# jianing-sun/Mask-YOLO

Measured on AMD Instinct MI355X. Metric: images/sec fwd+bwd, 224x224 Shapes batch 32, at 1 MI355X, higher is better.
Workload: dtype f32

## Files before the change

### include/myolo_hip_internal.h

```cpp
#ifndef MYOLO_HIP_INTERNAL_H
#define MYOLO_HIP_INTERNAL_H

#include "myolo_hip.h"

#ifdef __cplusplus
extern "C" {
#endif

int myolo_bn_frozen_coeffs_batched(const float* params, const float* stats, const int64_t* table, int nlayers, float* coeffs,
                                   void* stream);

int myolo_bn_act_bwd_frozen_post(const float* dy, const float* a_post, const float* gamma, const float* beta, const float* scale,
                                 float* dx, float* dgamma, float* dbeta, int64_t M, int C, int act,
                                 void* ws, size_t ws_bytes, void* stream);

int myolo_wprep_create(void* arena, size_t arena_bytes, void** handle);
int myolo_wprep_destroy(void* h);
int myolo_wprep_activate(void* h);
int myolo_wprep_count(void* h);
int myolo_wprep_invalidate(void* h);
int myolo_wprep_refresh(void* h, int first, int last, int max_idle, void* stream);
int myolo_wprep_stats(void* h, long long* hits, long long* misses, long long* bytes_used);
int myolo_wprep_overflows(void* h, long long* n);

// ... 49 lines not shown
                                   float* dx, float* dgamma, float* dbeta, int64_t M, int C, int act, const double* part, int nblk,
                                   void* ws, size_t ws_bytes, void* stream);

size_t myolo_wino63_plane_elems(int N, int C);
size_t myolo_wino63_u_elems(int Cin, int Cout);

int myolo_wino63_weight_transform(const float* w, float* U, int Cin, int Cout, void* stream);
int myolo_wino63_multiply(const float* V, const float* U, float* M, int N, int Cin, int Cout, void* stream);
int myolo_wino63_multiply_w(const float* V, const float* w, float* U_scratch, float* M, int N, int Cin, int Cout, void* stream);
int myolo_wino63_input_transform(const float* x, const float* scale, const float* shift, int act,
                                 float* keep, const int32_t* keep_sel, int keep_cap,
                                 float* V, int N, int C, void* stream);
int myolo_wino63_boundary(const float* M, const float* bias, const float* scale, const float* shift, int act,
                          float* y, float* keep, int keep_pre, const int32_t* keep_sel, int keep_cap,
                          float* Vn, int N, int C, void* stream);
int myolo_wino63_input_transform_roialign(const float* feature, const float* boxes, const int32_t* box_ind, float* V, int B, int FH, int FW,
                                          int C, int nb, void* stream);
size_t myolo_wino63_output_transform_bn_ws_bytes(int N, int C);
int myolo_wino63_output_transform_bn_stats(const float* M, const float* bias, float* y, int N, int C, const float* gamma, const float* beta,
                                           float* mean, float* var, float* scale, float* shift, float* moving_mean, float* moving_var,
                                           void* ws, size_t ws_bytes, void* stream);
size_t myolo_wino63_bwd_weight_ws_bytes(int N, int Cin, int Cout);
int myolo_wino63_bwd_weight_lazybn(const float* v_saved, const float* y_pre, const float* dy_compact, const int32_t* inv, const float* scale,
                                   const float* shift, const float* ka, const float* kb, int act, float* dw, int N, int Cin, int Cout,
                                   void* ws, size_t ws_bytes, void* stream);
int myolo_wino63_lazybn_transforms(const float* y_pre, const float* dy_compact, const int32_t* inv, const float* scale, const float* shift,
                                   const float* ka, const float* kb, int act, float* V, float* Q, int N, int C, void* stream);
size_t myolo_wino63_bwd_data_from_v_ws_bytes(int N, int Cin, int Cout);
int myolo_wino63_bwd_data_from_v(const float* V, const float* w, float* dx, int N, int Cin, int Cout, void* ws, size_t ws_bytes, void* stream);
size_t myolo_wino63_bwd_weight_from_q_ws_bytes(int N, int Cin, int Cout);
int myolo_wino63_bwd_weight_from_q(const float* v_saved, const float* Q, float* dw, int N, int Cin, int Cout, void* ws, size_t ws_bytes,
                                   void* stream);

int myolo_gemm_tn_bf16x6_planes(const float* A, const float* B, float* C, int nruns, const int64_t* rows, const int32_t* nq, int Ka, int N,
                                void* ws, size_t ws_bytes, void* stream);
int myolo_deconv2x2s2_bwd_weight_bf16x6(const float* x, const float* dy, float* dw, int N, int H, int W, int Cin, int Cout, void* ws, size_t ws_bytes,
                                        void* stream);

size_t myolo_wino63_bwd_data_ws_bytes(int N, int Cin, int Cout);
int myolo_wino63_bwd_data_lazybn(const float* y_pre, const float* dy_compact, const int32_t* inv, const float* scale, const float* shift,
                                 const float* ka, const float* kb, int act, const float* w, float* dx, int N, int Cin, int Cout, void* ws,
                                 size_t ws_bytes, void* stream);
int myolo_conv3x3s2_c3_affine_act_fwd(const float* x, const float* w, const float* scale, const float* shift, int act, float* y,
                                      int N, int H, int W, int Cout, void* stream);
size_t myolo_conv3x3s2_c3_bnstats_ws_bytes(int N, int H, int W, int Cout);
int myolo_conv3x3s2_c3_bnstats_fwd(const float* x, const float* w, float* y, const float* gamma, const float* beta, float* mean, float* var,
                                   float* scale, float* shift, float* moving_mean, float* moving_var, int N, int H, int W, int Cout, int phases,
                                   void* ws, size_t ws_bytes, void* stream);
size_t myolo_dwconv3x3_bnstats_ws_bytes(int N, int H, int W, int C, int stride);
int myolo_dwconv3x3_bnstats_fwd(const float* x, const float* in_scale, const float* in_shift, int in_act, const float* w, float* y,
                                const float* gamma, const float* beta, float* mean, float* var, float* scale, float* shift,
                                float* moving_mean, float* moving_var, int N, int H, int W, int C, int stride, int phases,
                                void* ws, size_t ws_bytes, void* stream);
int myolo_dwconv3x3_bwd_weight_affine_in(const float* x, const float* in_scale, const float* in_shift, int in_act, const float* dy, float* dw,
                                         int N, int H, int W, int C, int stride, void* ws, size_t ws_bytes, void* stream);
int    myolo_pwconv1x1_bnstats_ok(int Cin, int Cout);
size_t myolo_pwconv1x1_bnstats_ws_bytes(int64_t M, int Cin, int Cout);
int myolo_pwconv1x1_bnstats_fwd(const float* x, const float* in_scale, const float* in_shift, int in_act, const float* w, float* y,
                                const float* gamma, const float* beta, float* mean, float* var, float* scale, float* shift,
                                float* moving_mean, float* moving_var, int64_t M, int Cin, int Cout, int phases, void* ws, size_t ws_bytes, void* stream);
int myolo_pwconv1x1_bwd_weight_affine_in(const float* x, const float* in_scale, const float* in_shift, int in_act, const float* dy, float* dw,
                                         int64_t M, int Cin, int Cout, void* ws, size_t ws_bytes, void* stream);

int myolo_mask_bce_sel(const float* target_masks, const int32_t* target_class_ids, const float* pred, float loss_weight,
                       float* loss_out, float* dz_sel, int NR, int h, int w, int C, void* ws, size_t ws_bytes, void* stream);
size_t myolo_mask_head_out_bwd_sel_ws_bytes(int NR, int Cin);
// ... 128 lines not shown
```

### mask-yolo_amd/csrc/mem_kernels.hip

```cpp
#include "myolo_common.h"
#include <type_traits>
#include <stdlib.h>
#include <stdarg.h>
#include <string.h>

static thread_local char g_err[512] = "";
extern "C" void myolo_set_error(const char* fmt, ...)
{
    va_list ap;
    va_start(ap, fmt);
    vsnprintf(g_err, sizeof(g_err), fmt, ap);
    va_end(ap);
}
extern "C" const char* myolo_last_error_string(void) { return g_err; }
extern "C" int myolo_version(void) { return 213; }

static MyoloOptions default_options() { MyoloOptions o = {}; o.bn_fused_tf_variance = 1; o.tn_wgs = 224; return o; }
MyoloOptions g_myolo_opt = default_options();
static int* option_slot(const char* name)
{
    static const struct { const char* n; int MyoloOptions::*m; } tab[] = {
        {"gemm_generic", &MyoloOptions::gemm_generic}, {"no_splitk", &MyoloOptions::no_splitk}, {"bf16_no256", &MyoloOptions::bf16_no256},
        {"bf16_force256", &MyoloOptions::bf16_force256}, {"bf16_no_c3", &MyoloOptions::bf16_no_c3}, {"bf16_no_loopn", &MyoloOptions::bf16_no_loopn},
        {"bf16_mask_valu", &MyoloOptions::bf16_mask_valu}, {"bf16_mask_nofin", &MyoloOptions::bf16_mask_nofin},
        {"deconv_mask_legacy", &MyoloOptions::deconv_mask_legacy}, {"crop_bf16_legacy", &MyoloOptions::crop_bf16_legacy},
        {"tune0", &MyoloOptions::tune0}, {"wino_x6", &MyoloOptions::wino_x6}, {"wino_no_bt", &MyoloOptions::wino_no_bt},
        {"wino_no_mixed", &MyoloOptions::wino_no_mixed}, {"x6_no_half_tiles", &MyoloOptions::x6_no_half_tiles},
        {"w63_legacy", &MyoloOptions::w63_legacy}, {"pw_x6_min_rows", &MyoloOptions::pw_x6_min_rows}, {"deconv_no_x6", &MyoloOptions::deconv_no_x6},
        {"pw_no_smallm", &MyoloOptions::pw_no_smallm}, {"pw_no_x6", &MyoloOptions::pw_no_x6}, {"tn_no_x6", &MyoloOptions::tn_no_x6},
        {"tn_wgs", &MyoloOptions::tn_wgs}, {"tn_x6_legacy", &MyoloOptions::tn_x6_legacy}, {"no_trunk_fusion", &MyoloOptions::no_trunk_fusion},
        {"bn_fused_tf_variance", &MyoloOptions::bn_fused_tf_variance},
    };
    if (!name) return nullptr;
    for (const auto& e : tab)
        if (strcmp(e.n, name) == 0) return &(g_myolo_opt.*(e.m));
    return nullptr;
}
extern "C" int myolo_set_option(const char* name, int value)
{
    int* s = option_slot(name);
    MYOLO_REQUIRE(s, "set_option: unknown option '%s'", name ? name : "(null)");
    *s = value;
    return MYOLO_OK;
}
extern "C" int myolo_get_option(const char* name, int* value)
{
    int* s = option_slot(name);
    MYOLO_REQUIRE(s && value, "get_option: unknown option '%s'", name ? name : "(null)");
    *value = *s;
    return MYOLO_OK;
}

#include <vector>
struct WPrepEntry {
    const void* w; int kind; long long d0, d1, d2;
    size_t off, bytes;
    unsigned long long gen;
    unsigned long long last_use;
    std::function<void(void*, hipStream_t)> run;
};
struct WPrep {
    char* arena; size_t cap, used;
    unsigned long long gen;
// ... 3439 lines not shown
```

### mask-yolo_amd/csrc/myolo_common.h

```cpp
#pragma once
#include <hip/hip_runtime.h>
#include <stdint.h>
#include <stdio.h>
#include "../../include/myolo_hip_internal.h"

extern "C" void myolo_set_error(const char* fmt, ...);

struct MyoloOptions {
    int gemm_generic;
    int no_splitk;
    int bf16_no256;
    int bf16_no_loopn;
    int bf16_mask_valu;
    int bf16_mask_nofin;
    int deconv_mask_legacy;
    int bf16_no_c3;
    int bf16_force256;
    int crop_bf16_legacy;
    int tune0;
    int wino_x6;
    int wino_no_bt;
    int wino_no_mixed;
    int x6_no_half_tiles;
    int w63_legacy;
    int pw_x6_min_rows;
    int deconv_no_x6;
    int pw_no_smallm;
    int pw_no_x6;
    int tn_no_x6;
    int tn_wgs;
    int tn_x6_legacy;
    int no_trunk_fusion;
    int bn_fused_tf_variance;
};
extern MyoloOptions g_myolo_opt;

#define MYOLO_REQUIRE(cond, ...)                                   \
    do {                                                           \
        if (!(cond)) {                                             \
            myolo_set_error(__VA_ARGS__);                          \
            return MYOLO_EINVAL;                                   \
        }                                                          \
    } while (0)

#define MYOLO_NEED_WS(bytes)                                                         \
    do {                                                                             \
        if ((size_t)(bytes) > ws_bytes || (ws == nullptr && (bytes) > 0)) {          \
            myolo_set_error("%s: workspace too small (%zu needed, %zu given)",       \
                            __func__, (size_t)(bytes), ws_bytes);                    \
            return MYOLO_EWORKSPACE;                                                 \
        }                                                                            \
    } while (0)

#define MYOLO_CHECK_LAUNCH()                                                         \
    do {                                                                             \
        hipError_t e__ = hipGetLastError();                                          \
        if (e__ != hipSuccess) {                                                     \
            myolo_set_error("%s: launch failed: %s", __func__, hipGetErrorString(e__)); \
            return MYOLO_ELAUNCH;                                                    \
        }                                                                            \
    } while (0)

#include <functional>
enum { WP_TRANSPOSE = 1, WP_X6_SPLIT = 2, WP_WINO63_U = 3, WP_WINO43_U = 4 };
// ... 47 lines not shown
```

### mask-yolo_amd/csrc/wino_mm.hip

```cpp
#include "myolo_common.h"

typedef float f32x16 __attribute__((ext_vector_type(16)));
typedef unsigned int u32x4 __attribute__((ext_vector_type(4)));

#define MM_BM 128
#define MM_BN 256
#define MM_BK 16
#define MM_LD 20
#define MM_OOB 0x7fffff00u

struct MMRun {
    long long rows;
    long long a_off;
    long long b_off;
    long long c_off;
    long long tile0;
    int mtiles;
    int nq;
};
struct MMArgs {
    const float* A;
    const float* Bt;
    float* C;
    int K, N;
// ... 994 lines not shown
        else hipLaunchKernelGGL(wino_mm_x6_kernel<MM_EP_PLAIN>, dim3((unsigned)tiles), dim3(256), 0, s, a);
    } else {
        if (!b_is_nk) {
            hipLaunchKernelGGL(mm_transpose_kn_kernel, dim3((N + 31) / 32, (K + 31) / 32), dim3(256), 0, s, B, (float*)ws, K, N);
            a.Bt = (const float*)ws;
        } else a.Bt = B;
        hipLaunchKernelGGL(wino_mm_kernel<MM_EP_PLAIN>, dim3((unsigned)tiles), dim3(256), 0, s, a);
    }
    MYOLO_CHECK_LAUNCH();
    return MYOLO_OK;
}

#define TN_T 256
struct TNRun {
    long long rows;
    long long a_off, b_off;
    long long rows_per_split;
    long long unit0;
    int plane0;
    int nq;
    int splits;
};
struct TNArgs {
    const float* a_scale;
    const float* a_shift;
    int a_act;
    int gH, gW, gCo;
    const float* A;
    const float* B;
    float* part;
    float* C;
    int Ka, N;
    int nruns;
    int tiles_k, tiles_n;
    long long nunits;
    long long unit_base;
    int tune;
    TNRun run[4];
};

template <bool AG = false, bool UNI = true>
__global__ __launch_bounds__(512, 1) void wino_tn_x6_kernel(TNArgs p)
{
    __shared__ __attribute__((aligned(16))) unsigned char Ls[2][2][TN_T * X6_REC];

    const int tid = threadIdx.x, lane = tid & 63, wave = tid >> 6;
    const int wm = wave >> 2, wn = wave & 3, half = lane >> 5, l31 = lane & 31;
    const int ntile = p.tiles_k * p.tiles_n;
  const long long bid = p.unit_base + blockIdx.x;
  {
    const long long pair = bid / ntile;
    const int tile = (int)(bid - pair * ntile);
    const int kat = tile / p.tiles_n, nt = tile - kat * p.tiles_n;
    int ri = 0;
#pragma unroll
    for (int k = 1; k < 4; ++k)
        if (k < p.nruns && pair >= p.run[k].unit0) ri = k;
    const TNRun& R = p.run[ri];
    const long long local = pair - R.unit0;
    const int z = (int)(local / R.splits), sp = (int)(local - (long long)z * R.splits);
    const long long r0 = (long long)sp * R.rows_per_split;
    long long r1 = r0 + R.rows_per_split;
    if (r1 > R.rows) r1 = R.rows;
    const long long nrows = r1 > r0 ? r1 - r0 : 0;
    const int nk = (int)((nrows + MM_BK - 1) / MM_BK);

// ... 116 lines not shown
                for (int pc = 0; pc < 3; ++pc) fn[pc] = *reinterpret_cast<const bf16x8*>(la + afr + (t + 1) * 32 * X6_REC + pc * 32);
            }
#ifdef MM_X6_TUNE
            if (!(p.tune & 4))
#endif
#pragma unroll
            for (int u = 0; u < 2; ++u) {
                acc[t][u] = __builtin_amdgcn_mfma_f32_32x32x16_bf16(fa[0], fb[u][2], acc[t][u], 0, 0, 0);
                acc[t][u] = __builtin_amdgcn_mfma_f32_32x32x16_bf16(fa[2], fb[u][0], acc[t][u], 0, 0, 0);
                acc[t][u] = __builtin_amdgcn_mfma_f32_32x32x16_bf16(fa[1], fb[u][1], acc[t][u], 0, 0, 0);
                acc[t][u] = __builtin_amdgcn_mfma_f32_32x32x16_bf16(fa[0], fb[u][1], acc[t][u], 0, 0, 0);
                acc[t][u] = __builtin_amdgcn_mfma_f32_32x32x16_bf16(fa[1], fb[u][0], acc[t][u], 0, 0, 0);
                acc[t][u] = __builtin_amdgcn_mfma_f32_32x32x16_bf16(fa[0], fb[u][0], acc[t][u], 0, 0, 0);
            }
            if (t == 0 && more) split_store(cur ^ 1, 0);
            if (t == 1 && more) split_store(cur ^ 1, 1);
            if (t == 2 && c + 2 < nk) gload();
            if (t < 3) { fa[0] = fn[0]; fa[1] = fn[1]; fa[2] = fn[2]; }
        }
        __syncthreads();
    }
    float* Pp = p.part + pair * (long long)p.Ka * p.N + ((long long)kat * TN_T + wm * 128) * p.N + nt * TN_T + wn * 64 + l31;
#pragma unroll
    for (int t = 0; t < 4; ++t)
#pragma unroll
        for (int r = 0; r < 16; ++r) {
            const int row = t * 32 + (r & 3) + 8 * (r >> 2) + 4 * half;
#pragma unroll
            for (int u = 0; u < 2; ++u) Pp[(long long)row * p.N + u * 32] = acc[t][u][r];
        }
  }
}

__global__ __launch_bounds__(256) void tn_x6_reduce_kernel(TNArgs p)
{
    const int plane = blockIdx.y;
    int ri = 0;
#pragma unroll
    for (int k = 1; k < 4; ++k)
        if (k < p.nruns && plane >= p.run[k].plane0) ri = k;
    const TNRun& R = p.run[ri];
    const long long n4 = (long long)p.Ka * p.N / 4;
    const long long i = (long long)blockIdx.x * 256 + threadIdx.x;
    if (i >= n4) return;
    const float4* src = reinterpret_cast<const float4*>(p.part) + (R.unit0 + (long long)(plane - R.plane0) * R.splits) * n4 + i;
    float4 s = make_float4(0.f, 0.f, 0.f, 0.f);
    int k = 0;
    for (; k + 4 <= R.splits; k += 4) {
        const float4 a = src[(long long)k * n4], b = src[(long long)(k + 1) * n4], c = src[(long long)(k + 2) * n4], d = src[(long long)(k + 3) * n4];
        s.x += a.x; s.y += a.y; s.z += a.z; s.w += a.w;
        s.x += b.x; s.y += b.y; s.z += b.z; s.w += b.w;
        s.x += c.x; s.y += c.y; s.z += c.z; s.w += c.w;
        s.x += d.x; s.y += d.y; s.z += d.z; s.w += d.w;
    }
    for (; k < R.splits; ++k) {
        const float4 a = src[(long long)k * n4];
        s.x += a.x; s.y += a.y; s.z += a.z; s.w += a.w;
    }
    reinterpret_cast<float4*>(p.C)[(long long)plane * n4 + i] = s;
}

bool myolo_gemm_tn_x6_ok(int Ka, int N) { return g_myolo_opt.wino_x6 && !g_myolo_opt.tn_no_x6 && Ka >= TN_T && (Ka % TN_T) == 0 && N >= TN_T && (N % TN_T) == 0; }

static long long tn_x6_plan(int nruns, const long long* rows, const int* nq, int Ka, int N, TNArgs* a)
{
    const int ntile = (Ka / TN_T) * (N / TN_T);
    long long total_rows = 0;
    for (int r = 0; r < nruns; ++r) total_rows += rows[r] * nq[r];
    const long long target_units = 3 * (g_myolo_opt.tn_wgs > 0 ? g_myolo_opt.tn_wgs : 256);
    long long rps = ((total_rows * ntile + target_units - 1) / target_units + MM_BK - 1) / MM_BK * MM_BK;
    if (rps < 8 * MM_BK) rps = 8 * MM_BK;
    long long pairs = 0;
    for (int iter = 0; iter < 64; ++iter) {
        pairs = 0;
        for (int r = 0; r < nruns; ++r) pairs += (long long)nq[r] * ((rows[r] + rps - 1) / rps);
        if (pairs * ntile <= target_units || rps >= total_rows) break;
        rps += MM_BK;
    }
    if (a) {
        long long unit = 0;
        int plane = 0;
        a->nruns = 0;
        for (int r = 0; r < nruns; ++r) {
            if (rows[r] <= 0 || nq[r] <= 0) continue;
            TNRun& R = a->run[a->nruns++];
            R.rows = rows[r]; R.nq = nq[r]; R.plane0 = plane; R.unit0 = unit;
            R.splits = (int)((rows[r] + rps - 1) / rps);
            R.rows_per_split = ((rows[r] + R.splits - 1) / R.splits + MM_BK - 1) / MM_BK * MM_BK;
            unit += (long long)R.nq * R.splits;
            plane += nq[r];
        }
    }
    return pairs;
}

static long long tn_x6_grid(long long nunits) { return g_myolo_opt.tn_wgs > 0 && nunits > g_myolo_opt.tn_wgs ? g_myolo_opt.tn_wgs : nunits; }

template <bool AG>
static void tn_x6_launch(TNArgs& a, hipStream_t s)
{
    for (long long base = 0, g = tn_x6_grid(a.nunits); base < a.nunits; base += g) {
        a.unit_base = base;
        const unsigned n = (unsigned)(a.nunits - base < g ? a.nunits - base : g);
        if (g_myolo_opt.tn_x6_legacy) hipLaunchKernelGGL((wino_tn_x6_kernel<AG, false>), dim3(n), dim3(512), 0, s, a);
        else hipLaunchKernelGGL((wino_tn_x6_kernel<AG, true>), dim3(n), dim3(512), 0, s, a);
    }
}

size_t myolo_gemm_tn_x6_ws_bytes(int nruns, const long long* rows, const int* nq, int Ka, int N)
{
    return align256((size_t)tn_x6_plan(nruns, rows, nq, Ka, N, nullptr) * Ka * N * sizeof(float));
}

int myolo_gemm_tn_x6_runs(const float* A, const float* B, float* C, int nruns, const long long* rows, const long long* a_off, const long long* b_off,
                          const int* nq, int Ka, int N, void* part, size_t part_bytes, hipStream_t s,
                          const float* a_scale, const float* a_shift, int a_act)
{
    if (nruns < 0 || nruns > 4 || Ka < TN_T || (Ka % TN_T) || N < TN_T || (N % TN_T) || ((uintptr_t)A & 15) || ((uintptr_t)B & 15) || ((uintptr_t)C & 15)) {
        myolo_set_error("gemm_tn_x6_runs: needs Ka %% %d == 0, N %% %d == 0, <= 4 runs, 16-byte aligned operands", TN_T, TN_T);
        return MYOLO_EINVAL;
    }
    TNArgs a{};
    a.A = A; a.B = B; a.C = C; a.part = (float*)part; a.Ka = Ka; a.N = N; a.tiles_k = Ka / TN_T; a.tiles_n = N / TN_T;
    a.a_scale = a_scale; a.a_shift = a_shift; a.a_act = a_act;
    const long long pairs = tn_x6_plan(nruns, rows, nq, Ka, N, &a);
    if ((size_t)pairs * Ka * N * sizeof(float) > part_bytes || !part) {
        myolo_set_error("gemm_tn_x6_runs: workspace too small (%zu needed, %zu given)", (size_t)pairs * Ka * N * sizeof(float), part_bytes);
        return MYOLO_EWORKSPACE;
    }
    int k = 0, planes = 0;
    for (int r = 0; r < nruns; ++r) {
        if (rows[r] <= 0 || nq[r] <= 0) continue;
        if ((a_off[r] | b_off[r]) & 3) { myolo_set_error("gemm_tn_x6_runs: run offsets must be multiples of 4 elements"); return MYOLO_EINVAL; }
        a.run[k].a_off = a_off[r]; a.run[k].b_off = b_off[r];
        planes += nq[r];
        ++k;
    }
    if (pairs <= 0) return MYOLO_OK;
    a.nunits = pairs * a.tiles_k * a.tiles_n;
#ifdef MM_X6_TUNE
    a.tune = g_myolo_opt.tune0;
#endif
    tn_x6_launch<false>(a, s);
    const long long n4 = (long long)Ka * N / 4;
    hipLaunchKernelGGL(tn_x6_reduce_kernel, dim3((unsigned)((n4 + 255) / 256), planes), dim3(256), 0, s, a);
    return MYOLO_OK;
}

extern "C" int myolo_gemm_tn_bf16x6_planes(const float* A, const float* B, float* C, int nruns, const int64_t* rows, const int32_t* nq, int Ka, int N,
                                           void* ws, size_t ws_bytes, void* stream)
{
    MYOLO_REQUIRE(A && B && C && rows && nq && nruns >= 0 && nruns <= 4 && Ka > 0 && N > 0, "gemm_tn_bf16x6_planes: bad arguments");
    long long r[4], ao[4], bo[4], at = 0;
    int q[4];
    for (int k = 0; k < nruns; ++k) {
        MYOLO_REQUIRE(rows[k] >= 0 && nq[k] >= 0, "gemm_tn_bf16x6_planes: negative run");
        r[k] = rows[k]; q[k] = nq[k]; ao[k] = at * Ka; bo[k] = at * N;
        at += rows[k] * nq[k];
    }
    const int rc = myolo_gemm_tn_x6_runs(A, B, C, nruns, r, ao, bo, q, Ka, N, ws, ws_bytes, (hipStream_t)stream);
    if (rc) return rc;
    MYOLO_CHECK_LAUNCH();
    return MYOLO_OK;
}

bool myolo_pw_x6_ok(int K, int N) { return g_myolo_opt.wino_x6 && !g_myolo_opt.pw_no_x6 && K >= 256 && (K % MM_BK) == 0 && (N % MM_BN) == 0; }
size_t myolo_pw_x6_split_bytes(int K, int N) { return align256((size_t)K * N * 6); }
int myolo_pw_x6_fwd(const float* x, const float* in_scale, const float* in_shift, int in_act, const float* w, float* y, double* stat,
                    long long M, int K, int N, void* split, hipStream_t s)
{
    MMArgs a{};
    a.A = x; a.C = y; a.K = K; a.N = N; a.nruns = 1;
    a.a_scale = in_scale; a.a_shift = in_shift; a.a_act = in_act; a.stat = stat;
#ifdef MM_X6_TUNE
    a.tune = g_myolo_opt.tune0;
#endif
    MMRun& R = a.run[0];
    R.rows = M; R.a_off = 0; R.b_off = 0; R.c_off = 0; R.nq = 1; R.tile0 = 0;
    R.mtiles = (int)((M + MM_BM - 1) / MM_BM);
// ... 15 lines not shown
{
    const int K = Cin, N = 4 * Co;
    MMArgs a{};
    a.A = x; a.C = y; a.K = K; a.N = N; a.nruns = 1; a.bias = bias; a.H = H; a.W = W; a.Co = Co; a.a_act = act;
#ifdef MM_X6_TUNE
    a.tune = g_myolo_opt.tune0;
#endif
    MMRun& R = a.run[0];
    R.rows = M; R.nq = 1; R.mtiles = (int)((M + MM_BM - 1) / MM_BM);
    a.Bt = x6_split_weights(w, split, K, N, 0, s);
    hipLaunchKernelGGL((wino_mm_x6_kernel<MM_EP_DECONV, false, MM_A_PLAIN>), dim3((unsigned)((long long)R.mtiles * (N / MM_BN))), dim3(256), 0, s, a);
    return MYOLO_OK;
}
int myolo_deconv_x6_bwd_data(const float* dy, const float* w, float* dx, long long M, int H, int W, int Cin, int Co, void* split, hipStream_t s)
{
    const int K = 4 * Co, N = Cin;
    MMArgs a{};
    a.A = dy; a.C = dx; a.K = K; a.N = N; a.nruns = 1; a.H = H; a.W = W; a.Co = Co;
#ifdef MM_X6_TUNE
    a.tune = g_myolo_opt.tune0;
#endif
    MMRun& R = a.run[0];
    R.rows = M; R.nq = 1; R.mtiles = (int)((M + MM_BM - 1) / MM_BM);
    a.Bt = x6_split_weights(w, split, K, N, 1, s);
    hipLaunchKernelGGL((wino_mm_x6_kernel<MM_EP_PLAIN, false, MM_A_DECONV>), dim3((unsigned)((long long)R.mtiles * (N / MM_BN))), dim3(256), 0, s, a);
    return MYOLO_OK;
}


size_t myolo_deconv_x6_bwd_weight_ws_bytes(long long M, int Cin, int Co)
{
    const long long rows[1] = {M};
    const int nq[1] = {1};
    return myolo_gemm_tn_x6_ws_bytes(1, rows, nq, 4 * Co, Cin);
}
int myolo_deconv_x6_bwd_weight(const float* x, const float* dy, float* dw, long long M, int H, int W, int Cin, int Co, void* part, size_t part_bytes,
                               hipStream_t s)
{
    const int Ka = 4 * Co, N = Cin;
    TNArgs a{};
    a.A = dy; a.B = x; a.C = dw; a.part = (float*)part; a.Ka = Ka; a.N = N; a.tiles_k = Ka / TN_T; a.tiles_n = N / TN_T;
    a.gH = H; a.gW = W; a.gCo = Co;
    const long long rows[1] = {M};
    const int nq[1] = {1};
    const long long pairs = tn_x6_plan(1, rows, nq, Ka, N, &a);
    if ((size_t)pairs * Ka * N * sizeof(float) > part_bytes || !part) {
        myolo_set_error("deconv_x6_bwd_weight: workspace too small (%zu needed, %zu given)", (size_t)pairs * Ka * N * sizeof(float), part_bytes);
        return MYOLO_EWORKSPACE;
    }
    a.run[0].a_off = 0; a.run[0].b_off = 0;
    a.nunits = pairs * a.tiles_k * a.tiles_n;
    tn_x6_launch<true>(a, s);
    const long long n4 = (long long)Ka * N / 4;
    hipLaunchKernelGGL(tn_x6_reduce_kernel, dim3((unsigned)((n4 + 255) / 256), 1), dim3(256), 0, s, a);
    return MYOLO_OK;
}

extern "C" int myolo_deconv2x2s2_bwd_weight_bf16x6(const float* x, const float* dy, float* dw, int N, int H, int W, int Cin, int Cout, void* ws, size_t ws_bytes,
                                                   void* stream)
{
    MYOLO_REQUIRE(x && dy && dw && N > 0 && H > 0 && W > 0 && Cin > 0 && Cout > 0 && (Cin % TN_T) == 0 && ((4 * Cout) % TN_T) == 0 &&
                  (((uintptr_t)x | (uintptr_t)dy | (uintptr_t)dw) & 15) == 0, "deconv2x2s2_bwd_weight_bf16x6: needs Cin %% 256 == 0, 4 Cout %% 256 == 0, 16-byte aligned operands");
    const int rc = myolo_deconv_x6_bwd_weight(x, dy, dw, (long long)N * H * W, H, W, Cin, Cout, ws, ws_bytes, (hipStream_t)stream);
    if (rc) return rc;
    MYOLO_CHECK_LAUNCH();
    return MYOLO_OK;
}
```

### mask-yolo_amd/myolo/_ext.py

```python
import ctypes
import os

import torch

_LIB = None
_HERE = os.path.dirname(os.path.abspath(__file__))
LIB_PATH = os.environ.get("MYOLO_LIB") or os.path.join(_HERE, "_lib", "libmyolo_hip.so")

P, I, L, F, Z, D = ctypes.c_void_p, ctypes.c_int, ctypes.c_int64, ctypes.c_float, ctypes.c_size_t, ctypes.c_double

SIGS = {
    "myolo_conv3x3s2_c3_fwd": [P, P, P, I, I, I, I, P],
    "myolo_conv3x3s2_c3_affine_act_fwd": [P, P, P, P, I, P, I, I, I, I, P],
    "myolo_conv3x3s2_c3_bwd_weight": [P, P, P, I, I, I, I, P, Z, P],
    "myolo_dwconv3x3_fwd": [P, P, P, I, I, I, I, I, P],
    "myolo_dwconv3x3_affine_act_fwd": [P, P, P, P, I, P, I, I, I, I, I, P],
    "myolo_dwconv3x3_bwd_data": [P, P, P, I, I, I, I, I, P],
    "myolo_dwconv3x3_bwd_data_bnsums": [P, P, P, I, I, I, I, I, P, P, P, P, P, I, P, I, P],
    "myolo_bn_act_bwd_from_partials": [P, P, P, P, P, P, P, P, P, L, I, I, P, I, P, Z, P],
    "myolo_dwconv3x3_bwd_weight": [P, P, P, I, I, I, I, I, P, Z, P],
    "myolo_pwconv1x1_fwd": [P, P, P, P, L, I, I, P, Z, P],
    "myolo_pwconv1x1_affine_act_fwd": [P, P, P, P, I, P, L, I, I, P, Z, P],
    "myolo_bn_frozen_coeffs_batched": [P, P, P, I, P, P],
    "myolo_pwconv1x1_bwd_data": [P, P, P, L, I, I, P, Z, P],
# ... 120 lines not shown
}


def load():
    global _LIB
    if _LIB is not None:
        return _LIB
    if not os.path.exists(LIB_PATH):
        raise RuntimeError("libmyolo_hip.so not built (%s): run `python __graft_entry__.py` "
                           "(hipcc --offload-arch=gfx950); there is no fallback path" % LIB_PATH)
    lib = ctypes.CDLL(LIB_PATH)
    for name, argtypes in SIGS.items():
        fn = getattr(lib, name)
        fn.argtypes = argtypes
        fn.restype = ctypes.c_int
    lib.myolo_version.restype = ctypes.c_int
    lib.myolo_last_error_string.restype = ctypes.c_char_p
    lib.myolo_workspace_bytes.argtypes = [L, I, I]
    lib.myolo_workspace_bytes.restype = Z
    lib.myolo_conv3x3_wino_ws_bytes.argtypes = [I, I, I, I, I, I]
    lib.myolo_conv3x3_wino_ws_bytes.restype = Z
    lib.myolo_matmul_f32_ws_bytes.argtypes = [I, I, I, I]
    lib.myolo_matmul_f32_ws_bytes.restype = Z
    lib.myolo_conv3x3s2_c3_bnstats_ws_bytes.argtypes = [I, I, I, I]
    lib.myolo_conv3x3s2_c3_bnstats_ws_bytes.restype = Z
    lib.myolo_dwconv3x3_bnstats_ws_bytes.argtypes = [I, I, I, I, I]
    lib.myolo_dwconv3x3_bnstats_ws_bytes.restype = Z
    lib.myolo_dwconv3x3_bwd_weight_ws_bytes.argtypes = [I, I, I, I, I]
    lib.myolo_dwconv3x3_bwd_weight_ws_bytes.restype = Z
    lib.myolo_pwconv1x1_bnstats_ws_bytes.argtypes = [L, I, I]
    lib.myolo_pwconv1x1_bnstats_ws_bytes.restype = Z
    lib.myolo_pwconv1x1_bnstats_ok.argtypes = [I, I]
    lib.myolo_pwconv1x1_bnstats_ok.restype = I
    lib.myolo_wino_plane_elems.argtypes = [I, I, I, I]
    lib.myolo_wino_plane_elems.restype = Z
    lib.myolo_wino_u_elems.argtypes = [I, I]
    lib.myolo_wino_u_elems.restype = Z
    lib.myolo_wino63_u_elems.argtypes = [I, I]
    lib.myolo_wino63_u_elems.restype = Z
    lib.myolo_wino63_plane_elems.argtypes = [I, I]
    lib.myolo_wino63_plane_elems.restype = Z
    lib.myolo_wino63_bwd_data_ws_bytes.argtypes = [I, I, I]
    lib.myolo_wino63_bwd_data_ws_bytes.restype = Z
    lib.myolo_conv3x3_wino63_ws_bytes.argtypes = [I, I, I, I]
    lib.myolo_conv3x3_wino63_ws_bytes.restype = Z
    lib.myolo_wino63_bwd_weight_ws_bytes.argtypes = [I, I, I]
    lib.myolo_wino63_bwd_weight_ws_bytes.restype = Z
    for fn in (lib.myolo_wino63_bwd_data_from_v_ws_bytes, lib.myolo_wino63_bwd_weight_from_q_ws_bytes):
        fn.argtypes = [I, I, I]
        fn.restype = Z
    lib.myolo_wino63_output_transform_bn_ws_bytes.argtypes = [I, I]
    lib.myolo_wino63_output_transform_bn_ws_bytes.restype = Z
    lib.myolo_wino63_ok.argtypes = [I, I, I, I]
    lib.myolo_wino63_ok.restype = I
    lib.myolo_deconv2x2s2_mask_ws_bytes.argtypes = [I, I, I, I, I, I]
    lib.myolo_deconv2x2s2_mask_ws_bytes.restype = Z
    lib.myolo_wino_output_transform_bn_ws_bytes.argtypes = [I]
    lib.myolo_wino_output_transform_bn_ws_bytes.restype = Z
    lib.myolo_mask_head_out_bwd_sel_ws_bytes.argtypes = [I, I]
    lib.myolo_mask_head_out_bwd_sel_ws_bytes.restype = Z
    lib.myolo_wprep_create.argtypes = [P, Z, P]
    lib.myolo_wprep_create.restype = I
    for fn in (lib.myolo_wprep_destroy, lib.myolo_wprep_activate, lib.myolo_wprep_invalidate):
        fn.argtypes = [P]
        fn.restype = I
    lib.myolo_wprep_count.argtypes = [P]
    lib.myolo_wprep_count.restype = I
    lib.myolo_dwconv3x3_bwd_data_bnsums_rows.argtypes = [I, I, I, I, I]
    lib.myolo_dwconv3x3_bwd_data_bnsums_rows.restype = I
    lib.myolo_conv7x7s2_c3_ws_bytes.argtypes = [I, I, I, I]
    lib.myolo_conv7x7s2_c3_ws_bytes.restype = Z
    lib.myolo_augment_batch_ws_bytes.argtypes = [I, I]
    lib.myolo_augment_batch_ws_bytes.restype = Z
    lib.myolo_mosaic_batch_ws_bytes.argtypes = [I, I]
    lib.myolo_mosaic_batch_ws_bytes.restype = Z
    lib.myolo_copy_paste_batch_ws_bytes.argtypes = [I, I]
    lib.myolo_copy_paste_batch_ws_bytes.restype = Z
    lib.myolo_resize_images_ws_bytes.argtypes = [I]
    lib.myolo_resize_images_ws_bytes.restype = Z
    lib.myolo_rle_masks_ws_bytes.argtypes = [I, I, I]
    lib.myolo_rle_masks_ws_bytes.restype = Z
    lib.myolo_contour_masks_ws_bytes.argtypes = [I, I, I, I, L]
    lib.myolo_contour_masks_ws_bytes.restype = Z
    lib.myolo_anchor_kmeans_ws_bytes.argtypes = [L, I]
    lib.myolo_anchor_kmeans_ws_bytes.restype = Z
    lib.myolo_wprep_refresh.argtypes = [P, I, I, I, P]
    lib.myolo_wprep_refresh.restype = I
    _LIB = lib
    return lib


def exported_symbols():
    return list(SIGS) + ["myolo_version", "myolo_last_error_string", "myolo_workspace_bytes", "myolo_conv3x3_wino_ws_bytes", "myolo_wino_plane_elems", "myolo_wino_u_elems", "myolo_wino63_u_elems", "myolo_wino63_plane_elems", "myolo_wino63_ok", "myolo_wino63_bwd_data_ws_bytes", "myolo_wino63_bwd_weight_ws_bytes", "myolo_wino63_bwd_data_from_v_ws_bytes", "myolo_wino63_bwd_weight_from_q_ws_bytes", "myolo_wino63_output_transform_bn_ws_bytes", "myolo_conv3x3_wino63_ws_bytes", "myolo_matmul_f32_ws_bytes", "myolo_conv3x3s2_c3_bnstats_ws_bytes", "myolo_dwconv3x3_bnstats_ws_bytes", "myolo_dwconv3x3_bwd_weight_ws_bytes",
                              "myolo_pwconv1x1_bnstats_ws_bytes", "myolo_pwconv1x1_bnstats_ok",
                              "myolo_deconv2x2s2_mask_ws_bytes", "myolo_wino_output_transform_bn_ws_bytes", "myolo_mask_head_out_bwd_sel_ws_bytes",
                              "myolo_dwconv3x3_bwd_data_bnsums_rows", "myolo_wprep_create", "myolo_wprep_destroy", "myolo_wprep_activate", "myolo_wprep_invalidate", "myolo_wprep_count", "myolo_wprep_refresh",
                              "myolo_conv7x7s2_c3_ws_bytes", "myolo_augment_batch_ws_bytes", "myolo_mosaic_batch_ws_bytes", "myolo_copy_paste_batch_ws_bytes",
                              "myolo_resize_images_ws_bytes",
                              "myolo_rle_masks_ws_bytes", "myolo_contour_masks_ws_bytes", "myolo_anchor_kmeans_ws_bytes"]


def ptr(t):
    if t is None:
        return None
    assert t.is_cuda and t.is_contiguous(), "C-ABI needs contiguous device tensors"
    return t.data_ptr()


def stream():
    return torch.cuda.current_stream().cuda_stream


def call(name, *args):
    lib = load()
    rc = getattr(lib, name)(*args)
    if rc != 0:
        raise RuntimeError("%s failed (%d): %s" % (name, rc, lib.myolo_last_error_string().decode()))


class WeightPrep(object):

    def __init__(self, device, arena_bytes=768 << 20):
        self.arena = torch.empty(int(arena_bytes), dtype=torch.uint8, device=device)
        h = ctypes.c_void_p(0)
        call("myolo_wprep_create", self.arena.data_ptr(), self.arena.numel(), ctypes.byref(h))
        self.h = h.value
# ... 280 lines not shown
```

Baseline: 1707.

## Add small-tile split-K TN bf16x6 GEMM path for few-row weight-gradient problems

Adds a 128x128-tile variant of the bf16x6 TN GEMM kernel, double-buffered through LDS, plus a planner heuristic that selects it when there are few planes and little total row work. Smaller tiles and a capped rows-per-split produce more work units, which is meant to fill the GPU on small weight-gradient GEMMs and cut partial-buffer traffic. The path is on by default and is excluded from deconv. It also adds a workspace-size query export and an optional census print. The tradeoff is that smaller tiles give less reuse, and the selection thresholds are hand-picked.

```diff
diff --git a/include/myolo_hip_internal.h b/include/myolo_hip_internal.h
--- a/include/myolo_hip_internal.h
+++ b/include/myolo_hip_internal.h
@@ -105,6 +105,7 @@
 int myolo_wino63_bwd_weight_from_q(const float* v_saved, const float* Q, float* dw, int N, int Cin, int Cout, void* ws, size_t ws_bytes,
                                    void* stream);
 
+size_t myolo_gemm_tn_bf16x6_planes_ws_bytes(int nruns, const int64_t* rows, const int32_t* nq, int Ka, int N);
 int myolo_gemm_tn_bf16x6_planes(const float* A, const float* B, float* C, int nruns, const int64_t* rows, const int32_t* nq, int Ka, int N,
                                 void* ws, size_t ws_bytes, void* stream);
 int myolo_deconv2x2s2_bwd_weight_bf16x6(const float* x, const float* dy, float* dw, int N, int H, int W, int Cin, int Cout, void* ws, size_t ws_bytes,
diff --git a/mask-yolo_amd/csrc/mem_kernels.hip b/mask-yolo_amd/csrc/mem_kernels.hip
--- a/mask-yolo_amd/csrc/mem_kernels.hip
+++ b/mask-yolo_amd/csrc/mem_kernels.hip
@@ -15,7 +15,7 @@
 extern "C" const char* myolo_last_error_string(void) { return g_err; }
 extern "C" int myolo_version(void) { return 213; }
 
-static MyoloOptions default_options() { MyoloOptions o = {}; o.bn_fused_tf_variance = 1; o.tn_wgs = 224; return o; }
+static MyoloOptions default_options() { MyoloOptions o = {}; o.bn_fused_tf_variance = 1; o.tn_wgs = 224; o.tn_x6_small = 1; return o; }
 MyoloOptions g_myolo_opt = default_options();
 static int* option_slot(const char* name)
 {
@@ -28,7 +28,8 @@
         {"wino_no_mixed", &MyoloOptions::wino_no_mixed}, {"x6_no_half_tiles", &MyoloOptions::x6_no_half_tiles},
         {"w63_legacy", &MyoloOptions::w63_legacy}, {"pw_x6_min_rows", &MyoloOptions::pw_x6_min_rows}, {"deconv_no_x6", &MyoloOptions::deconv_no_x6},
         {"pw_no_smallm", &MyoloOptions::pw_no_smallm}, {"pw_no_x6", &MyoloOptions::pw_no_x6}, {"tn_no_x6", &MyoloOptions::tn_no_x6},
-        {"tn_wgs", &MyoloOptions::tn_wgs}, {"tn_x6_legacy", &MyoloOptions::tn_x6_legacy}, {"no_trunk_fusion", &MyoloOptions::no_trunk_fusion},
+        {"tn_wgs", &MyoloOptions::tn_wgs}, {"tn_x6_legacy", &MyoloOptions::tn_x6_legacy}, {"tn_x6_small", &MyoloOptions::tn_x6_small},
+        {"tn_x6_census", &MyoloOptions::tn_x6_census}, {"no_trunk_fusion", &MyoloOptions::no_trunk_fusion},
         {"bn_fused_tf_variance", &MyoloOptions::bn_fused_tf_variance},
     };
     if (!name) return nullptr;
diff --git a/mask-yolo_amd/csrc/myolo_common.h b/mask-yolo_amd/csrc/myolo_common.h
--- a/mask-yolo_amd/csrc/myolo_common.h
+++ b/mask-yolo_amd/csrc/myolo_common.h
@@ -30,6 +30,8 @@
     int tn_no_x6;
     int tn_wgs;
     int tn_x6_legacy;
+    int tn_x6_small;
+    int tn_x6_census;
     int no_trunk_fusion;
     int bn_fused_tf_variance;
 };
diff --git a/mask-yolo_amd/csrc/wino_mm.hip b/mask-yolo_amd/csrc/wino_mm.hip
--- a/mask-yolo_amd/csrc/wino_mm.hip
+++ b/mask-yolo_amd/csrc/wino_mm.hip
@@ -1050,6 +1050,7 @@
     float* C;
     int Ka, N;
     int nruns;
+    int small;
     int tiles_k, tiles_n;
     long long nunits;
     long long unit_base;
@@ -1232,6 +1233,137 @@
   }
 }
 
+#define TNS_T 128
+template <bool PRO, int ACT>
+__global__ __launch_bounds__(256, 2) void wino_tn_x6_small_kernel(TNArgs p)
+{
+    __shared__ __attribute__((aligned(16))) unsigned char Ls[2][2][TNS_T * X6_REC];
+
+    const int tid = threadIdx.x, lane = tid & 63, wave = tid >> 6;
+    const int wm = wave >> 1, wn = wave & 1, half = lane >> 5, l31 = lane & 31;
+    const int ntile = p.tiles_k * p.tiles_n;
+    const long long bid = blockIdx.x;
+    const long long pair = bid / ntile;
+    const int tile = (int)(bid - pair * ntile);
+    const int kat = tile / p.tiles_n, nt = tile - kat * p.tiles_n;
+    int ri = 0;
+#pragma unroll
+    for (int k = 1; k < 4; ++k)
+        if (k < p.nruns && pair >= p.run[k].unit0) ri = k;
+    const TNRun& R = p.run[ri];
+    const long long local = pair - R.unit0;
+    const int z = (int)(local / R.splits), sp = (int)(local - (long long)z * R.splits);
+    const long long r0 = (long long)sp * R.rows_per_split;
+    long long r1 = r0 + R.rows_per_split;
+    if (r1 > R.rows) r1 = R.rows;
+    const long long nrows = r1 > r0 ? r1 - r0 : 0;
+    const int nk = (int)((nrows + MM_BK - 1) / MM_BK);
+
+    const int op = __builtin_amdgcn_readfirstlane(tid >> 7), col = tid & (TNS_T - 1);
+    const int ld = op ? p.N : p.Ka;
+    const float* base = op ? p.B + R.b_off + ((long long)z * R.rows + r0) * p.N + nt * TNS_T
+                           : p.A + R.a_off + ((long long)z * R.rows + r0) * p.Ka + kat * TNS_T;
+    const __amdgpu_buffer_rsrc_t rs = mm_rsrc(base, (nrows * ld - (op ? nt : kat) * TNS_T) * 4);
+    const unsigned voff = (unsigned)col * 4u;
+    const unsigned rowb = (unsigned)ld * 4u;
+    unsigned soff = 0;
+    int chunk = 0;
+    auto gload = [&](float (&st)[16]) {
+        const unsigned so = chunk < nk ? soff : MM_OOB;
+#pragma unroll
+        for (int k = 0; k < 16; ++k) st[k] = __uint_as_float(__builtin_amdgcn_raw_buffer_load_b32(rs, (int)voff, (int)(so + (unsigned)k * rowb), 0));
+        soff += 16u * rowb;
+        ++chunk;
+    };
+    unsigned char* const wbase = &Ls[0][op][col * X6_REC];
+    const bool pro = PRO && op == 0;
+    const float csc = pro ? p.a_scale[kat * TNS_T + col] : 1.f, csh = pro ? p.a_shift[kat * TNS_T + col] : 0.f;
+    int arows = pro ? (int)nrows : 0;
+    if constexpr (PRO) asm("" : "+v"(arows));
+    auto split_store = [&](float (&st)[16], long long row0, int buf, int h) {
+        u32x4 p1, p2, p3;
+        if constexpr (PRO) {
+#pragma unroll
+            for (int j = 0; j < 8; ++j) {
+                const float x = st[8 * h + j];
+                st[8 * h + j] = (int)row0 + 8 * h + j < arows ? mm_act(fmaf(x, csc, csh), ACT) : x;
+            }
+        }
+#pragma unroll
+        for (int e = 0; e < 4; ++e) {
+            const float a0 = st[8 * h + 2 * e], a1 = st[8 * h + 2 * e + 1];
+            const float b0 = x6_rest(a0), b1 = x6_rest(a1);
+            p1[e] = x6_top(a0, a1);
+            p2[e] = x6_top(b0, b1);
+            p3[e] = x6_top(x6_rest(b0), x6_rest(b1));
+        }
+        unsigned char* w = wbase + buf * (2 * TNS_T * X6_REC) + h * 16;
+        *reinterpret_cast<u32x4*>(w) = p1;
+        *reinterpret_cast<u32x4*>(w + 32) = p2;
+        *reinterpret_cast<u32x4*>(w + 64) = p3;
+    };
+    const int afr = (wm * 64 + l31) * X6_REC + half * 16;
+    const int bfr = (wn * 64 + l31) * X6_REC + half * 16;
+
+    f32x16 acc[2][2];
+#pragma unroll
+    for (int t = 0; t < 2; ++t)
+#pragma unroll
+        for (int u = 0; u < 2; ++u)
+#pragma unroll
+            for (int r = 0; r < 16; ++r) acc[t][u][r] = 0.f;
+
+    float s0[16], s1[16];
+    gload(s0);
+    gload(s1);
+    split_store(s0, 0, 0, 0);
+    split_store(s0, 0, 0, 1);
+    gload(s0);
+    __syncthreads();
+    auto step = [&](int c, float (&sn)[16]) {
+        const int cur = c & 1;
+        const unsigned char* la = &Ls[cur][0][0];
+        const unsigned char* lb = &Ls[cur][1][0];
+        bf16x8 fb[2][3], fa[2][3];
+#pragma unroll
+        for (int u = 0; u < 2; ++u)
+#pragma unroll
+            for (int pc = 0; pc < 3; ++pc) fb[u][pc] = *reinterpret_cast<const bf16x8*>(lb + bfr + u * 32 * X6_REC + pc * 32);
+#pragma unroll
+        for (int t = 0; t < 2; ++t)
+#pragma unroll
+            for (int pc = 0; pc < 3; ++pc) fa[t][pc] = *reinterpret_cast<const bf16x8*>(la + afr + t * 32 * X6_REC + pc * 32);
+#pragma unroll
+        for (int t = 0; t < 2; ++t) {
+#pragma unroll
+            for (int u = 0; u < 2; ++u) {
+                acc[t][u] = __builtin_amdgcn_mfma_f32_32x32x16_bf16(fa[t][0], fb[u][2], acc[t][u], 0, 0, 0);
+                acc[t][u] = __builtin_amdgcn_mfma_f32_32x32x16_bf16(fa[t][2], fb[u][0], acc[t][u], 0, 0, 0);
+                acc[t][u] = __builtin_amdgcn_mfma_f32_32x32x16_bf16(fa[t][1], fb[u][1], acc[t][u], 0, 0, 0);
+                acc[t][u] = __builtin_amdgcn_mfma_f32_32x32x16_bf16(fa[t][0], fb[u][1], acc[t][u], 0, 0, 0);
+                acc[t][u] = __builtin_amdgcn_mfma_f32_32x32x16_bf16(fa[t][1], fb[u][0], acc[t][u], 0, 0, 0);
+                acc[t][u] = __builtin_amdgcn_mfma_f32_32x32x16_bf16(fa[t][0], fb[u][0], acc[t][u], 0, 0, 0);
+            }
+            split_store(sn, (long long)(c + 1) * MM_BK, cur ^ 1, t);
+        }
+        gload(sn);
+        __syncthreads();
+    };
+    for (int c = 0; c < nk; c += 2) {
+        step(c, s1);
+        if (c + 1 < nk) step(c + 1, s0);
+    }
+    float* Pp = p.part + pair * (long long)p.Ka * p.N + ((long long)kat * TNS_T + wm * 64) * p.N + nt * TNS_T + wn * 64 + l31;
+#pragma unroll
+    for (int t = 0; t < 2; ++t)
+#pragma unroll
+        for (int r = 0; r < 16; ++r) {
+            const int row = t * 32 + (r & 3) + 8 * (r >> 2) + 4 * half;
+#pragma unroll
+            for (int u = 0; u < 2; ++u) Pp[(long long)row * p.N + u * 32] = acc[t][u][r];
+        }
+}
+
 __global__ __launch_bounds__(256) void tn_x6_reduce_kernel(TNArgs p)
 {
     const int plane = blockIdx.y;
@@ -1262,25 +1394,45 @@
 
 bool myolo_gemm_tn_x6_ok(int Ka, int N) { return g_myolo_opt.wino_x6 && !g_myolo_opt.tn_no_x6 && Ka >= TN_T && (Ka % TN_T) == 0 && N >= TN_T && (N % TN_T) == 0; }
 
-static long long tn_x6_plan(int nruns, const long long* rows, const int* nq, int Ka, int N, TNArgs* a)
-{
-    const int ntile = (Ka / TN_T) * (N / TN_T);
+static bool tn_x6_few_rows(int nruns, const long long* rows, const int* nq, int Ka, int N, bool ag)
+{
+    if (ag || g_myolo_opt.tn_x6_small <= 0) return false;
+    long long total_rows = 0, planes = 0;
+    for (int r = 0; r < nruns; ++r) {
+        if (rows[r] <= 0 || nq[r] <= 0) continue;
+        if (rows[r] > 32768) return false;
+        total_rows += rows[r] * nq[r];
+        planes += nq[r];
+    }
+    return planes > 0 && planes < 64 && total_rows * (Ka / TN_T) * (N / TN_T) < 24ll * MM_BK * 3 * 224;
+}
+
+static long long tn_x6_plan(int nruns, const long long* rows, const int* nq, int Ka, int N, TNArgs* a, bool ag = false)
+{
+    const bool small = tn_x6_few_rows(nruns, rows, nq, Ka, N, ag);
+    const int T = small ? TNS_T : TN_T;
+    const int ntile = (Ka / T) * (N / T);
     long long total_rows = 0;
     for (int r = 0; r < nruns; ++r) total_rows += rows[r] * nq[r];
-    const long long target_units = 3 * (g_myolo_opt.tn_wgs > 0 ? g_myolo_opt.tn_wgs : 256);
+    const long long target_units = small ? 512 : 3 * (g_myolo_opt.tn_wgs > 0 ? g_myolo_opt.tn_wgs : 256);
+    const long long floor_rows = (small ? 4 : 8) * MM_BK;
+    const long long cap_rows = 16 * MM_BK;
     long long rps = ((total_rows * ntile + target_units - 1) / target_units + MM_BK - 1) / MM_BK * MM_BK;
-    if (rps < 8 * MM_BK) rps = 8 * MM_BK;
+    if (rps < floor_rows) rps = floor_rows;
+    if (small && rps > cap_rows) rps = cap_rows;
     long long pairs = 0;
     for (int iter = 0; iter < 64; ++iter) {
         pairs = 0;
         for (int r = 0; r < nruns; ++r) pairs += (long long)nq[r] * ((rows[r] + rps - 1) / rps);
-        if (pairs * ntile <= target_units || rps >= total_rows) break;
+        if (pairs * ntile <= target_units || rps >= total_rows || (small && rps >= cap_rows)) break;
         rps += MM_BK;
     }
     if (a) {
         long long unit = 0;
         int plane = 0;
         a->nruns = 0;
+        a->small = small;
+        a->tiles_k = Ka / T; a->tiles_n = N / T;
         for (int r = 0; r < nruns; ++r) {
             if (rows[r] <= 0 || nq[r] <= 0) continue;
             TNRun& R = a->run[a->nruns++];
@@ -1307,6 +1459,16 @@
     }
 }
 
+static void tn_x6_census(const char* who, const TNArgs& a, long long pairs)
+{
+    if (!g_myolo_opt.tn_x6_census) return;
+    fprintf(stderr, "tn_x6_census %s form=%d Ka=%d N=%d units=%lld pairs=%lld partial_bytes=%lld runs=", who, a.small ? TNS_T : TN_T, a.Ka, a.N,
+            pairs * a.tiles_k * a.tiles_n, pairs, pairs * a.Ka * a.N * 4);
+    for (int k = 0; k < a.nruns; ++k)
+        fprintf(stderr, "%s%lldx%d:%dx%lld", k ? "," : "", a.run[k].rows, a.run[k].nq, a.run[k].splits, a.run[k].rows_per_split);
+    fprintf(stderr, "\n");
+}
+
 size_t myolo_gemm_tn_x6_ws_bytes(int nruns, const long long* rows, const int* nq, int Ka, int N)
 {
     return align256((size_t)tn_x6_plan(nruns, rows, nq, Ka, N, nullptr) * Ka * N * sizeof(float));
@@ -1321,7 +1483,7 @@
         return MYOLO_EINVAL;
     }
     TNArgs a{};
-    a.A = A; a.B = B; a.C = C; a.part = (float*)part; a.Ka = Ka; a.N = N; a.tiles_k = Ka / TN_T; a.tiles_n = N / TN_T;
+    a.A = A; a.B = B; a.C = C; a.part = (float*)part; a.Ka = Ka; a.N = N;
     a.a_scale = a_scale; a.a_shift = a_shift; a.a_act = a_act;
     const long long pairs = tn_x6_plan(nruns, rows, nq, Ka, N, &a);
     if ((size_t)pairs * Ka * N * sizeof(float) > part_bytes || !part) {
@@ -1338,13 +1500,33 @@
     }
     if (pairs <= 0) return MYOLO_OK;
     a.nunits = pairs * a.tiles_k * a.tiles_n;
+    tn_x6_census("gemm_tn_x6_runs", a, pairs);
 #ifdef MM_X6_TUNE
     a.tune = g_myolo_opt.tune0;
 #endif
-    tn_x6_launch<false>(a, s);
+    if (a.small) {
+        const dim3 grid((unsigned)a.nunits);
+        if (!a_scale) hipLaunchKernelGGL((wino_tn_x6_small_kernel<false, 0>), grid, dim3(256), 0, s, a);
+        else if (a_act == MYOLO_ACT_RELU6) hipLaunchKernelGGL((wino_tn_x6_small_kernel<true, MYOLO_ACT_RELU6>), grid, dim3(256), 0, s, a);
+        else if (a_act == MYOLO_ACT_RELU) hipLaunchKernelGGL((wino_tn_x6_small_kernel<true, MYOLO_ACT_RELU>), grid, dim3(256), 0, s, a);
+        else hipLaunchKernelGGL((wino_tn_x6_small_kernel<true, MYOLO_ACT_NONE>), grid, dim3(256), 0, s, a);
+    } else
+        tn_x6_launch<false>(a, s);
     const long long n4 = (long long)Ka * N / 4;
     hipLaunchKernelGGL(tn_x6_reduce_kernel, dim3((unsigned)((n4 + 255) / 256), planes), dim3(256), 0, s, a);
     return MYOLO_OK;
+}
+
+extern "C" size_t myolo_gemm_tn_bf16x6_planes_ws_bytes(int nruns, const int64_t* rows, const int32_t* nq, int Ka, int N)
+{
+    if (!rows || !nq || nruns < 0 || nruns > 4 || Ka < TN_T || (Ka % TN_T) || N < TN_T || (N % TN_T)) return 0;
+    long long r[4];
+    int q[4];
+    for (int k = 0; k < nruns; ++k) {
+        if (rows[k] < 0 || nq[k] < 0) return 0;
+        r[k] = rows[k]; q[k] = nq[k];
+    }
+    return myolo_gemm_tn_x6_ws_bytes(nruns, r, q, Ka, N);
 }
 
 extern "C" int myolo_gemm_tn_bf16x6_planes(const float* A, const float* B, float* C, int nruns, const int64_t* rows, const int32_t* nq, int Ka, int N,
@@ -1426,24 +1608,25 @@
 {
     const long long rows[1] = {M};
     const int nq[1] = {1};
-    return myolo_gemm_tn_x6_ws_bytes(1, rows, nq, 4 * Co, Cin);
+    return align256((size_t)tn_x6_plan(1, rows, nq, 4 * Co, Cin, nullptr, true) * 4 * Co * Cin * sizeof(float));
 }
 int myolo_deconv_x6_bwd_weight(const float* x, const float* dy, float* dw, long long M, int H, int W, int Cin, int Co, void* part, size_t part_bytes,
                                hipStream_t s)
 {
     const int Ka = 4 * Co, N = Cin;
     TNArgs a{};
-    a.A = dy; a.B = x; a.C = dw; a.part = (float*)part; a.Ka = Ka; a.N = N; a.tiles_k = Ka / TN_T; a.tiles_n = N / TN_T;
+    a.A = dy; a.B = x; a.C = dw; a.part = (float*)part; a.Ka = Ka; a.N = N;
     a.gH = H; a.gW = W; a.gCo = Co;
     const long long rows[1] = {M};
     const int nq[1] = {1};
-    const long long pairs = tn_x6_plan(1, rows, nq, Ka, N, &a);
+    const long long pairs = tn_x6_plan(1, rows, nq, Ka, N, &a, true);
     if ((size_t)pairs * Ka * N * sizeof(float) > part_bytes || !part) {
         myolo_set_error("deconv_x6_bwd_weight: workspace too small (%zu needed, %zu given)", (size_t)pairs * Ka * N * sizeof(float), part_bytes);
         return MYOLO_EWORKSPACE;
     }
     a.run[0].a_off = 0; a.run[0].b_off = 0;
     a.nunits = pairs * a.tiles_k * a.tiles_n;
+    tn_x6_census("deconv_x6_bwd_weight", a, pairs);
     tn_x6_launch<true>(a, s);
     const long long n4 = (long long)Ka * N / 4;
     hipLaunchKernelGGL(tn_x6_reduce_kernel, dim3((unsigned)((n4 + 255) / 256), 1), dim3(256), 0, s, a);
diff --git a/mask-yolo_amd/myolo/_ext.py b/mask-yolo_amd/myolo/_ext.py
--- a/mask-yolo_amd/myolo/_ext.py
+++ b/mask-yolo_amd/myolo/_ext.py
@@ -176,6 +176,8 @@
     lib.myolo_pwconv1x1_bnstats_ws_bytes.restype = Z
     lib.myolo_pwconv1x1_bnstats_ok.argtypes = [I, I]
     lib.myolo_pwconv1x1_bnstats_ok.restype = I
+    lib.myolo_gemm_tn_bf16x6_planes_ws_bytes.argtypes = [I, P, P, I, I]
+    lib.myolo_gemm_tn_bf16x6_planes_ws_bytes.restype = Z
     lib.myolo_wino_plane_elems.argtypes = [I, I, I, I]
     lib.myolo_wino_plane_elems.restype = Z
     lib.myolo_wino_u_elems.argtypes = [I, I]
@@ -235,7 +237,7 @@
 
 
 def exported_symbols():
-    return list(SIGS) + ["myolo_version", "myolo_last_error_string", "myolo_workspace_bytes", "myolo_conv3x3_wino_ws_bytes", "myolo_wino_plane_elems", "myolo_wino_u_elems", "myolo_wino63_u_elems", "myolo_wino63_plane_elems", "myolo_wino63_ok", "myolo_wino63_bwd_data_ws_bytes", "myolo_wino63_bwd_weight_ws_bytes", "myolo_wino63_bwd_data_from_v_ws_bytes", "myolo_wino63_bwd_weight_from_q_ws_bytes", "myolo_wino63_output_transform_bn_ws_bytes", "myolo_conv3x3_wino63_ws_bytes", "myolo_matmul_f32_ws_bytes", "myolo_conv3x3s2_c3_bnstats_ws_bytes", "myolo_dwconv3x3_bnstats_ws_bytes", "myolo_dwconv3x3_bwd_weight_ws_bytes",
+    return list(SIGS) + ["myolo_version", "myolo_last_error_string", "myolo_workspace_bytes", "myolo_conv3x3_wino_ws_bytes", "myolo_wino_plane_elems", "myolo_wino_u_elems", "myolo_wino63_u_elems", "myolo_wino63_plane_elems", "myolo_wino63_ok", "myolo_wino63_bwd_data_ws_bytes", "myolo_wino63_bwd_weight_ws_bytes", "myolo_wino63_bwd_data_from_v_ws_bytes", "myolo_wino63_bwd_weight_from_q_ws_bytes", "myolo_wino63_output_transform_bn_ws_bytes", "myolo_conv3x3_wino63_ws_bytes", "myolo_matmul_f32_ws_bytes", "myolo_gemm_tn_bf16x6_planes_ws_bytes", "myolo_conv3x3s2_c3_bnstats_ws_bytes", "myolo_dwconv3x3_bnstats_ws_bytes", "myolo_dwconv3x3_bwd_weight_ws_bytes",
                               "myolo_pwconv1x1_bnstats_ws_bytes", "myolo_pwconv1x1_bnstats_ok",
                               "myolo_deconv2x2s2_mask_ws_bytes", "myolo_wino_output_transform_bn_ws_bytes", "myolo_mask_head_out_bwd_sel_ws_bytes",
                               "myolo_dwconv3x3_bwd_data_bnsums_rows", "myolo_wprep_create", "myolo_wprep_destroy", "myolo_wprep_activate", "myolo_wprep_invalidate", "myolo_wprep_count", "myolo_wprep_refresh",
```

Result: no change. 1699 (-0.4%).
